# zgcr/SimpleAICV_pytorch_training_examples

Measured on AMD Instinct MI355X. Metric: training images/sec/node, higher is better.
Workload: dtype bf16; 1 GPU; resnet50 3x224x224 synthetic training step (fwd+loss+bwd+all-reduce+optimizer), per-GPU batch 256; model=resnet50, global_batch=256, per_gpu_batch=256, parallelism=dp1, step_graph=True, bn_statistics=fixed-order partial rows, deterministic=True, loop=tools.scripts.train_classification, optimizer=SGD, param_groups=2

## Files before the change

### include/saicv_hip.h

```cpp
#ifndef SAICV_HIP_H
#define SAICV_HIP_H

#include <stddef.h>
#include <stdint.h>

#ifdef __cplusplus
extern "C" {
#endif

#define SAICV_BF16 0
#define SAICV_F32 1

typedef struct saicv_conv_desc {
    int N, H, W, C;
    int K, R, S;
    int stride, pad;
    int OH, OW;
    int dtype;
} saicv_conv_desc;

int saicv_version(void);
const char* saicv_last_error_string(void);

int saicv_set_deterministic(int on);
// ... 43 lines not shown
int saicv_linear_gelu_fwd_aux(int dtype, const void* x, const void* wf, const float* bias, void* y_dact, void* y_act, int M,
                              int K, int N, void* stream);
int saicv_linear_dgrad_mul(int dtype, const void* dy, const void* wd, const void* factor, void* dx, int M, int K, int N,
                           void* stream);
int saicv_linear_wgrad(int dtype, const void* dy, const void* x, float* dw, float* dbias, int M, int K, int N,
                       void* stream);
int saicv_conv2d_dgrad_add(const saicv_conv_desc* d, const void* dy, const void* wd, const void* addend, void* dx,
                           void* stream);
typedef struct saicv_dgrad_fuse {
    const void* addend;
    const void* addend_gate;
    const void* bn_y;
    const void* bn_mask;
    const float* bn_mean;
    const float* bn_invstd;
    float* part_g;
    float* part_gx;
    int part_rows;
    int reserved;
} saicv_dgrad_fuse;
int saicv_conv2d_dgrad_stat_rows(const saicv_conv_desc* d);
int saicv_conv2d_dgrad_fused(const saicv_conv_desc* d, const void* dy, const void* wd, const saicv_dgrad_fuse* f, void* dx,
                             void* stream);
#define SAICV_PLAN_CONV_FWD 0
#define SAICV_PLAN_CONV_DGRAD 1
#define SAICV_PLAN_CONV_WGRAD 2
#define SAICV_PLAN_LINEAR_FWD 3
#define SAICV_PLAN_LINEAR_DGRAD 4
#define SAICV_PLAN_LINEAR_WGRAD 5
typedef struct saicv_plan_query {
    int op;
    saicv_conv_desc conv;
    int dtype, M, K, N;
    int out_f32, bias, stats, addend, row_scale, bn_sums, act_mode;
} saicv_plan_query;
#define SAICV_ROUTE_TILED 0
#define SAICV_ROUTE_PW_STREAM 1
#define SAICV_ROUTE_PW3_STREAM 2
#define SAICV_ROUTE_TN 3
typedef struct saicv_plan {
    int route;
    int tile;
    int bm, bn;
    int kc8;
    int plain;
    int out_f32;
// ... 275 lines not shown
```

### simpleaicv_pytorch_training_examples_amd/_lib.py

```python
import ctypes
import os
from ctypes import POINTER, Structure, c_char_p, c_double, c_float, c_int, c_long, c_size_t, c_void_p

import torch

HERE = os.path.dirname(os.path.abspath(__file__))
LIB_PATH = os.path.join(HERE, 'libsaicv_hip.so')

BF16, F32 = 0, 1


class ConvDesc(Structure):
    _fields_ = [('N', c_int), ('H', c_int), ('W', c_int), ('C', c_int), ('K', c_int), ('R', c_int),
                ('S', c_int), ('stride', c_int), ('pad', c_int), ('OH', c_int), ('OW', c_int),
                ('dtype', c_int)]


_P = c_void_p
_PD = POINTER(ConvDesc)


class AttnDesc(Structure):
    _fields_ = [('q', _P), ('k', _P), ('v', _P),
                ('q_rs', c_long), ('k_rs', c_long), ('v_rs', c_long),
# ... 53 lines not shown
    'saicv_last_error_string': (c_char_p, []),
    'saicv_set_deterministic': (c_int, [c_int]),
    'saicv_get_deterministic': (c_int, []),
    'saicv_deterministic_prepare': (c_int, [_P]),
    'saicv_pack_input': (c_int, [c_int, _P, c_long, c_long, c_long, c_long, _P, c_int, c_int, c_int, c_int, c_int, _P]),
    'saicv_pack_weight': (c_int, [c_int, _P, c_long, c_long, c_long, c_long, c_int, c_int, c_int, c_int, c_int, c_int, _P, _P, _P]),
    'saicv_unpack_wgrad': (c_int, [_P, c_int, c_int, c_int, c_int, c_int, _P, c_long, c_long, c_long, c_long, c_int, _P]),
    'saicv_pack_weight_batched': (c_int, [c_int, _P, c_int, c_int, _P]),
    'saicv_pack_input_s2d': (c_int, [c_int, _P, c_long, c_long, c_long, c_long, _P, c_int, c_int, c_int, c_int, c_int, c_int, _P]),
    'saicv_pack_weight_s2d': (c_int, [c_int, _P, c_long, c_long, c_long, c_long, c_int, c_int, c_int, c_int, c_int, _P, _P]),
    'saicv_unpack_wgrad_s2d': (c_int, [_P, c_int, c_int, c_int, c_int, c_int, _P, c_long, c_long, c_long, c_long, c_int, _P]),
    'saicv_conv2d_stat_rows': (c_int, [_PD]),
    'saicv_conv2d_fwd': (c_int, [_PD, _P, _P, _P, _P, c_int, _P, _P, _P]),
    'saicv_conv2d_dgrad': (c_int, [_PD, _P, _P, _P, _P]),
    'saicv_conv2d_wgrad': (c_int, [_PD, _P, _P, _P, _P]),
    'saicv_conv2d_wgrad_bias': (c_int, [_PD, _P, _P, _P, _P, _P]),
    'saicv_colsum': (c_int, [c_int, _P, c_int, c_int, _P, _P]),
    'saicv_linear_fwd': (c_int, [c_int, _P, _P, _P, _P, c_int, c_int, c_int, c_int, _P, _P, c_int, _P]),
    'saicv_linear_dgrad': (c_int, [c_int, _P, _P, _P, c_int, c_int, c_int, _P, _P]),
    'saicv_linear_wgrad': (c_int, [c_int, _P, _P, _P, _P, c_int, c_int, c_int, _P]),
    'saicv_conv2d_dgrad_add': (c_int, [_PD, _P, _P, _P, _P, _P]),
    'saicv_conv2d_dgrad_stat_rows': (c_int, [_PD]),
    'saicv_conv2d_dgrad_fused': (c_int, [_PD, _P, _P, _PF, _P, _P]),
    'saicv_igemm_plan': (c_int, [POINTER(PlanQuery), POINTER(Plan)]),
    'saicv_conv2d_fwd_stats': (c_int, [_PD, _P, _P, _P, _P, _P, c_int, _P]),
    'saicv_bn_act_fwd_stats': (c_int, [c_int, _P, _P, _P, _P, _P, c_int, c_double, _P, _P, _P, _P, c_double, c_double, _P, _P, _P,
                                       c_size_t, c_int, c_int, _P, _P]),
    'saicv_bn_act_fwd_join': (c_int, [c_int, _P, _P, _P, _P, _P, _P, _P, _P, _P, c_int, c_double, _P, _P, _P, _P, c_double, c_double,
                                      _P, _P, _P, c_size_t, c_int, c_int, _P, _P]),
    'saicv_bn_act_bwd_inline': (c_int, [c_int, _P, _P, _P, _P, _P, _P, _P, _P, c_int, _P, _P, _P, _P, c_size_t, c_int, c_int,
                                        c_int, _P]),
    'saicv_bn_act_bwd_from_partials': (c_int, [c_int, _P, _P, _P, _P, _P, _P, _P, _P, c_int, _P, _P, _P, _P, c_size_t, c_int,
                                               c_int, c_int, _P, _P]),
    'saicv_row_scale': (c_int, [c_int, _P, _P, _P, c_size_t, c_int, c_int, _P]),
    'saicv_bn_ws_floats': (c_size_t, [c_int]),
    'saicv_bn_finalize_fwd': (c_int, [_P, _P, c_int, c_int, c_double, _P, _P, _P, _P, c_double, c_double, _P, _P, _P, _P, _P, _P, _P]),
    'saicv_bn_eval_coeffs': (c_int, [c_int, _P, _P, _P, _P, c_double, _P, _P, _P]),
    'saicv_bn_act_fwd': (c_int, [c_int, _P, _P, _P, _P, _P, c_size_t, c_int, c_int, _P, _P]),
    'saicv_bn_bwd_ws_floats': (c_size_t, [c_size_t, c_int, c_int]),
    'saicv_bn_act_bwd': (c_int, [c_int, _P, _P, _P, _P, _P, _P, _P, _P, _P, _P, _P, c_size_t, c_int, c_int, c_int, _P, _P]),
    'saicv_maxpool_fwd': (c_int, [c_int, _P, _P, _P, c_int, c_int, c_int, c_int, c_int, c_int, c_int, c_int, c_int, _P]),
    'saicv_maxpool_bwd': (c_int, [c_int, _P, _P, _P, c_int, c_int, c_int, c_int, c_int, c_int, c_int, c_int, c_int, _P]),
    'saicv_bn_relu_maxpool_fwd': (c_int, [c_int, _P, _P, _P, _P, _P] + [c_int] * 9 + [_P]),
    'saicv_bn_relu_maxpool_bwd_ws_floats': (c_size_t, [c_int]),
    'saicv_bn_relu_maxpool_bwd': (c_int, [c_int, _P, _P, _P, _P, _P, _P, _P, _P, _P, _P, _P, c_int, _P] + [c_int] * 9 + [_P]),
    'saicv_avgpool_fwd': (c_int, [c_int, _P, _P, c_int, c_int, c_int, _P]),
# ... 162 lines not shown
```

### simpleaicv_pytorch_training_examples_amd/build.py

```python
import os
import subprocess
import sys

HERE = os.path.dirname(os.path.abspath(__file__))
CSRC = os.path.join(HERE, 'csrc')
LIB = os.path.join(HERE, 'libsaicv_hip.so')
SOURCES = ['igemm.hip', 'pwstream.hip', 'bn.hip', 'pool.hip', 'loss.hip', 'pack.hip', 'optim.hip', 'muon.hip', 'tfm.hip', 'attn_stream.hip', 'maskloss.hip', 'sam.hip', 'samtail.hip', 'semseg.hip', 'salient.hip', 'input.hip', 'dwconv.hip', 'elemwise.hip', 'detloss.hip', 'groupnorm.hip', 'comm.hip', 'det.hip', 'capi.hip']
FLAGS = ['--offload-arch=gfx950', '-O3', '-std=c++17', '-fPIC', '-munsafe-fp-atomics',
         '-Wno-unused-result', '-Wno-unused-value']
EXTRA_FLAGS = {'attn_stream.hip': ['-fno-honor-nans', '-Wno-inline-asm']}


def _hipcc():
    for cand in (os.environ.get('HIPCC'), '/opt/rocm/bin/hipcc', 'hipcc'):
        if cand and (os.path.isabs(cand) and os.path.exists(cand) or not os.path.isabs(cand)):
            return cand
    return 'hipcc'


def _stale(out, deps):
    if not os.path.exists(out):
        return True
    t = os.path.getmtime(out)
    return any(os.path.getmtime(d) > t for d in deps if os.path.exists(d))


def build(force=False, verbose=True):
    hipcc = _hipcc()
    headers = [os.path.join(CSRC, h) for h in os.listdir(CSRC) if h.endswith('.h')]
    headers.append(os.path.join(os.path.dirname(HERE), 'include', 'saicv_hip.h'))
# ... 35 lines not shown
```

### simpleaicv_pytorch_training_examples_amd/csrc/bn.hip

```cpp
#include "common.h"
#include "saicv_internal.h"

namespace {


constexpr int kMaxBlocks = 1024;

__global__ __launch_bounds__(256) void bn_reduce_partials_kernel(const float* __restrict__ a,
                                                                 const float* __restrict__ b, int P,
                                                                 int C, float* __restrict__ oa,
                                                                 float* __restrict__ ob, int rows_per) {
    const int c = blockIdx.x * 64 + (threadIdx.x & 63);
    const int ty = threadIdx.x >> 6;
    const int p0 = blockIdx.y * rows_per;
    const int p1 = min(P, p0 + rows_per);
    float sa = 0.f, sb = 0.f;
    if (c < C) {
        float a4[4] = {0.f, 0.f, 0.f, 0.f}, b4[4] = {0.f, 0.f, 0.f, 0.f};
        int p = p0 + ty;
        for (; p + 12 < p1; p += 16) {
#pragma unroll
            for (int u = 0; u < 4; ++u) {
                a4[u] += a[(size_t)(p + 4 * u) * C + c];
                b4[u] += b[(size_t)(p + 4 * u) * C + c];
// ... 553 lines not shown
    SAICV_REQUIRE(part_g && part_gx && rows >= 1 && rows <= 64, "bn_bwd_inline: partial sums missing");
    SAICV_REQUIRE(!relu || relu_mask != nullptr, "bn_bwd_inline: relu needs the sign mask");
    const BnBwdInline inl = {part_g, part_gx, rows, (float)M, gamma, mean, invstd, dgamma, dbeta, accumulate};
    if (dtype == SAICV_DTYPE_BF16) return bn_bwd_inline_t<bf16_t>(dz, (const uint8_t*)relu_mask, y, dy, dres, M, C, relu, inl, st);
    return bn_bwd_inline_t<float>(dz, (const uint8_t*)relu_mask, y, dy, dres, M, C, relu, inl, st);
}

int bn_bwd_from_partials(int dtype, const void* dz, const void* relu_mask, const void* y, const float* gamma,
                         const float* mean, const float* invstd, const float* part_g, const float* part_gx, int rows,
                         void* dy, void* dres, float* dgamma, float* dbeta, size_t M, int C, int relu, int accumulate,
                         float* ws, hipStream_t st) {
    const uint8_t* mask = (const uint8_t*)relu_mask;
    const int n = dtype == SAICV_DTYPE_BF16 ? 8 : 4;
    SAICV_REQUIRE(C % n == 0, "bn_bwd_from_partials: C=%d must be a multiple of %d", C, n);
    SAICV_REQUIRE(part_g != nullptr && part_gx != nullptr && rows > 0, "bn_bwd_from_partials: partial sums missing");
    SAICV_REQUIRE(!relu || mask != nullptr, "bn_bwd_from_partials: relu needs the sign mask");
    if (dtype == SAICV_DTYPE_BF16)
        return bn_bwd_t<bf16_t>(dz, nullptr, mask, y, gamma, mean, invstd, dy, dres, dgamma, dbeta, M, C, relu, accumulate, ws, st,
                                part_g, part_gx, rows);
    return bn_bwd_t<float>(dz, nullptr, mask, y, gamma, mean, invstd, dy, dres, dgamma, dbeta, M, C, relu, accumulate, ws, st,
                           part_g, part_gx, rows);
}

int bn_bwd(int dtype, const void* dz, const void* z, const void* relu_mask, const void* y, const float* gamma,
           const float* mean, const float* invstd, void* dy, void* dres, float* dgamma, float* dbeta,
           size_t M, int C, int relu, int accumulate, float* ws, hipStream_t st) {
    const uint8_t* mask = (const uint8_t*)relu_mask;
    const int n = dtype == SAICV_DTYPE_BF16 ? 8 : 4;
    SAICV_REQUIRE(C % n == 0, "bn_bwd: C=%d must be a multiple of %d", C, n);
    SAICV_REQUIRE(!relu || z != nullptr || mask != nullptr, "bn_bwd: relu needs the forward output z or its sign mask");
    if (dtype == SAICV_DTYPE_BF16)
        return bn_bwd_t<bf16_t>(dz, z, mask, y, gamma, mean, invstd, dy, dres, dgamma, dbeta, M, C, relu, accumulate, ws, st);
    return bn_bwd_t<float>(dz, z, mask, y, gamma, mean, invstd, dy, dres, dgamma, dbeta, M, C, relu, accumulate, ws, st);
}

}
```

### simpleaicv_pytorch_training_examples_amd/csrc/capi.hip

```cpp
#include <stdarg.h>
#include <stdio.h>
#include <string.h>

#include "common.h"
#include "saicv_internal.h"
#include "../../include/saicv_hip.h"

namespace saicv {

static thread_local char g_err[512] = "";

void set_error(const char* fmt, ...) {
    va_list ap;
    va_start(ap, fmt);
    vsnprintf(g_err, sizeof(g_err), fmt, ap);
    va_end(ap);
}

int check_launch(const char* what) {
    const hipError_t e = hipGetLastError();
    if (e != hipSuccess) {
        set_error("%s: launch failed: %s", what, hipGetErrorString(e));
        return -2;
    }
// ... 216 lines not shown
                             void* stream) {
    if (check_desc(d, "saicv_conv2d_dgrad_fused")) return -1;
    if (!f) { set_error("saicv_conv2d_dgrad_fused: null fusion descriptor"); return -1; }
    const int M = d->N * d->H * d->W;
    EpiExtra ex;
    ex.addend = f->addend;
    ex.addend_gate = static_cast<const uint8_t*>(f->addend_gate);
    ex.bs_y = f->bn_y;
    ex.bs_mask = static_cast<const uint8_t*>(f->bn_mask);
    ex.bs_mean = f->bn_mean;
    ex.bs_invstd = f->bn_invstd;
    ex.bs_g = f->part_g;
    ex.bs_gx = f->part_gx;
    ex.stat_atomic_rows = f->part_rows;
    if (f->bn_y && d->stride > 1 && f->part_rows == 0) {
        const size_t bytes = (size_t)saicv_conv2d_dgrad_stat_rows(d) * d->C * sizeof(float);
        if (f->part_g) hipMemsetAsync(f->part_g, 0, bytes, S(stream));
        if (f->part_gx) hipMemsetAsync(f->part_gx, 0, bytes, S(stream));
    }
    return igemm_nt(d->dtype, 1, dy, wd, dx, nullptr, nullptr, nullptr, d->OH, d->OW, d->K, d->H, d->W,
                    d->R, d->S, d->stride, d->pad, M, d->C, d->R * d->S * d->K, d->C, 0, S(stream),
                    (f->addend || f->bn_y) ? &ex : nullptr);
}
int saicv_igemm_plan(const saicv_plan_query* q, saicv_plan* plan) {
    if (!q || !plan) { set_error("saicv_igemm_plan: null argument"); return -1; }
    SAICV_REQUIRE(q->op >= SAICV_PLAN_CONV_FWD && q->op <= SAICV_PLAN_LINEAR_WGRAD, "saicv_igemm_plan: bad op %d", q->op);
    if (q->op <= SAICV_PLAN_CONV_WGRAD) {
        if (check_desc(&q->conv, "saicv_igemm_plan")) return -1;
    } else {
        SAICV_REQUIRE(q->dtype == SAICV_BF16 || q->dtype == SAICV_F32, "saicv_igemm_plan: bad dtype %d", q->dtype);
    }
    return igemm_plan(q, plan);
}
int saicv_row_scale(int dtype, const void* x, const float* scale, void* out, size_t rows, int row_len,
                    int rows_per_scale, void* stream) {
    return row_scale(dtype, x, scale, out, rows, row_len, rows_per_scale, S(stream));
}

int saicv_colsum(int dtype, const void* dy, int M, int N, float* dbias, void* stream) {
    return colsum(dtype, dy, M, N, dbias, S(stream));
}

size_t saicv_bn_ws_floats(int C) { return bn_ws_floats(C); }

int saicv_bn_finalize_fwd(const float* sum, const float* sq, int rows, int C, double count,
                          const float* gamma, const float* beta, float* running_mean,
// ... 291 lines not shown
```

### simpleaicv_pytorch_training_examples_amd/csrc/saicv_internal.h

```cpp
#pragma once
#include <hip/hip_runtime.h>

struct saicv_conv_desc;
struct saicv_plan_query;
struct saicv_plan;

namespace saicv {

void set_error(const char* fmt, ...);
int check_launch(const char* what);

int conv_stat_rows(const saicv_conv_desc* d);
struct EpiExtra {
    const void* addend = nullptr;
    const float* row_scale = nullptr;
    int rows_per_scale = 1;
    int act_mode = 0;
    void* out2 = nullptr;
    const uint8_t* addend_gate = nullptr;
    const void* bs_y = nullptr;
    const uint8_t* bs_mask = nullptr;
    const float* bs_mean = nullptr;
    const float* bs_invstd = nullptr;
    float* bs_g = nullptr;
    float* bs_gx = nullptr;
    int stat_atomic_rows = 0;
};
int conv_bwd_stat_rows(const saicv_conv_desc* d);
int igemm_nt(int dtype, int mode, const void* src, const void* wgt, void* out, const float* bias,
             float* stat_sum, float* stat_sq, int H, int W, int C, int OH, int OW, int R, int S,
             int stride, int pad, int M, int Nn, int Kd, int ldo, int out_f32, hipStream_t st,
             const EpiExtra* ex = nullptr);
int igemm_tn(int dtype, const void* dy, const void* src, float* dw, int H, int W, int C, int OH,
             int OW, int R, int S, int stride, int pad, int M, int Cout, int Kd, hipStream_t st,
             float* dbias = nullptr);

int igemm_plan(const saicv_plan_query* q, saicv_plan* out);

int pw_stream_blocks(int dtype, int M, int Nn, int Kd, bool fused_dgrad);
int pw_stream(int M, int Nn, int Kd, const void* src, const void* wgt, void* out, float* stat_sum, float* stat_sq,
              int stat_atomic_rows, const EpiExtra* ex, int stream_out, int blocks, hipStream_t st);
int pw3_stream_blocks(int dtype, int M, int Nn, int Kd);
int pw3_stream(int mode, int M, int H, int W, const void* src, const void* wgt, void* out, float* stat_sum, float* stat_sq,
               int stat_atomic_rows, const EpiExtra* ex, int stream_out, int blocks, hipStream_t st);

int window_partition(int dtype, const void* x, void* out, int B, int H, int W, int C, int ws, hipStream_t st);
int window_unpartition(int dtype, const void* win, const void* addend, void* out, int B, int H, int W, int C, int ws,
                       hipStream_t st);
int relpos_fwd(int dtype, const void* q, long q_rs, long q_bs, const float* tab_h, const float* tab_w, float* rel_h,
               float* rel_w, int B, int heads, int Sh, int Sw, hipStream_t st);
int relpos_bwd(int dtype, const void* q, void* dq, long q_rs, long q_bs, const float* tab_h, const float* tab_w,
               const float* d_rel_h, const float* d_rel_w, float* dtab_h, float* dtab_w, float* ws, int B, int heads, int Sh,
               int Sw, hipStream_t st);
size_t relpos_bwd_ws_floats(int Sh, int Sw);
int mask_loss_stats(int dtype, const void* logits, const float* targets, float* stats, int B, int M, size_t HW,
                    double alpha, double gamma, double thr, hipStream_t st);
int mask_loss_grad(int dtype, const void* logits, const float* targets, const float* coef, void* dlogits, int B, int M,
                   size_t HW, double alpha, double gamma, hipStream_t st);
int hyper_product_fwd(int dtype, const void* x, const void* hyper, void* out, int B, int Tm, int P, int C, hipStream_t st);
int hyper_product_bwd(int dtype, const void* x, const void* hyper, const void* dout, void* dx, float* dhyper, int B, int Tm,
                      int P, int C, hipStream_t st);
int upsample4_fwd(int dtype, const void* low, void* out, int planes, int h, int w, hipStream_t st);
int upsample4_bwd(int dtype, const void* dhi, void* dlow, int planes, int h, int w, hipStream_t st);
int mask_loss_stats_up4(int dtype, const void* low, const float* targets, float* stats, int B, int M, int h, int w,
                        double alpha, double gamma, double thr, hipStream_t st);
int mask_loss_grad_up4(int dtype, const void* low, const float* targets, const float* coef, void* dlow, int B, int M, int h,
                       int w, double alpha, double gamma, hipStream_t st);
size_t pixel_softmax_ce_ws_floats(size_t rows);
// ... 19 lines not shown
```

### simpleaicv_pytorch_training_examples_amd/ops.py

```python
import collections
import ctypes
import weakref

import torch

from . import _lib
from ._lib import ConvDesc, check, dtype_code, lib, ptr, require_gpu, stream

_weights_epoch = [0]


class KernelTimer:
    enabled = False
    only = None
    records = []
    PEAK_FLOPS, PEAK_BYTES = 2.5e15, 8.0e12

    @classmethod
    def begin(cls, tag=None):
        if not cls.enabled or (cls.only is not None and tag not in cls.only):
            return None
        e = torch.cuda.Event(enable_timing=True)
        e.record()
        return e
# ... 688 lines not shown
        fuse.bn_mean, fuse.bn_invstd = ptr(in_link.mean), ptr(in_link.invstd)
        fuse.part_g, fuse.part_gx = ptr(part[0]), ptr(part[1])
        in_link.part, in_link.rows = part, rows
    return fuse


def _pooled_bn_backward(ctx, st, dz, gamma, y, idx, mean, invstd):
    pk, ps, pp, poh, pow_, scale, shift = ctx.pool
    L = lib()
    dt, dev = y.dtype, y.device
    n, k, oh, ow = y.shape
    dy = _empty_nhwc(n, k, oh, ow, dt, dev)
    dgamma, dbeta, direct_bn = _bn_grad_buffers(gamma, ctx.beta_ref, k, dev)
    ws = torch.empty(L.saicv_bn_relu_maxpool_bwd_ws_floats(k), dtype=torch.float32, device=dev)
    t0 = KernelTimer.begin('bn_act_bwd')
    check(L.saicv_bn_relu_maxpool_bwd(dtype_code(dt), ptr(dz), ptr(idx), ptr(y), ptr(gamma), ptr(mean), ptr(invstd), ptr(scale),
                                      ptr(shift), ptr(dy), ptr(dgamma), ptr(dbeta), int(direct_bn), ptr(ws), n, oh, ow, k, poh, pow_,
                                      pk, ps, pp, st), 'bn_relu_maxpool_bwd')
    es = y.element_size()
    KernelTimer.end(t0, 'bn_act_bwd', 0, 3.0 * n * oh * ow * k * es + 2.0 * n * poh * pow_ * k * (es + 1))
    return (dy, None, None, None) if direct_bn else (dy, None, dgamma, dbeta)


class ConvBnActFn(torch.autograd.Function):

    _deferred = []

    @staticmethod
    def forward(ctx, x, weight, gamma, beta, residual, bn, stride, pad, relu, want_skip=False, pool=None, defer=False):
        if defer and (residual is not None or relu or want_skip or pool is not None):
            raise ValueError('a deferred BatchNorm-apply belongs to a plain convolution + BatchNorm shortcut')
        if pool is not None and (residual is not None or not relu or want_skip):
            raise ValueError('the fused max-pool follows a plain conv -> BatchNorm -> ReLU block')
        cs = _conv_stage(x, weight, gamma, beta, bn, stride, pad, ctx.needs_input_grad[0], pool is not None, defer)
        if pool is not None:
            return _pooled_tail(ctx, cs, weight, gamma, beta, stride, pad, pool)
        if defer:
            _remember(ctx, cs, weight, gamma, beta, stride, pad, False, False, applies_gate=bool(BN_FUSE and cs.training))
            ConvBnActFn._deferred.append((cs.scale, cs.shift))
            return cs.y
        return _apply_tail(ctx, cs, weight, gamma, beta, stride, pad, relu, residual, want_skip)

    @staticmethod
    def backward(ctx, dz, dskip=None):
        x, weight, gamma, y, mask, mean, invstd = ctx.saved_tensors
        stride, pad, relu, has_res, training, d, wd = ctx.cfg
        if not training:
            raise NotImplementedError('backward through eval-mode BatchNorm is not implemented')
        dt, st = y.dtype, stream()
        gate_in = _take_gate(dz)
        dz0 = dz
        dz = _nhwc(dz, dt)
        if ctx.pool is not None:
            dy, dres, dgamma, dbeta = _pooled_bn_backward(ctx, st, dz, gamma, y, mask, mean, invstd)
        else:
            dy, dres, dgamma, dbeta = _bn_act_backward(ctx, st, dz, dz is dz0, gate_in, relu, has_res, gamma, y, mask, mean, invstd)
        n, k, oh, ow = y.shape
        M = n * oh * ow
        c = x.shape[1]
        flops = 2.0 * M * k * weight.shape[2] * weight.shape[3] * min(c, weight.shape[1])
        dx = dwt = None
        if ctx.needs_input_grad[0]:
            t0 = KernelTimer.begin('igemm_nt')
            gate = None
            if dskip is not None:
                gate = _take_gate(dskip)
                dskip = _nhwc(dskip, dt)
            in_link = ctx.in_link
            fuse = _dgrad_fuse(d, in_link, dskip, gate, y.device) if (gate is not None or in_link is not None) else None
            dx = _conv_data_grad(d, dy, weight, wd, x.shape, dt, st, fuse, dskip)
            if in_link is not None:
                in_link.dx, in_link.dx_version = dx, dx._version
            es = dy.element_size()
            px = float(n) * x.shape[2] * x.shape[3] * c
            nbytes = float(M) * k * es + float(k) * d.R * d.S * c * es + px * es
# ... 855 lines not shown
```

Baseline: 12550 images/s.

## Fuse bottleneck conv3 backward: BN-ReLU grad, dgrad and wgrad in one streaming kernel

Adds a streaming kernel for the 1x1 expansion conv of residual bottlenecks. In a single pass over each tile it applies the BN/ReLU backward coefficients to dz, computes the data gradient and accumulates the weight gradient, and optionally produces the next BN's partial sums. This removes separate BN-backward, dgrad and wgrad launches, along with the round trip of the intermediate dy tensor through memory. The trade-offs are a narrow eligibility condition, heavy register and LDS use per workgroup, and a deterministic cross-block reduction of the weight gradient.

```diff
diff --git a/include/saicv_hip.h b/include/saicv_hip.h
--- a/include/saicv_hip.h
+++ b/include/saicv_hip.h
@@ -89,6 +89,13 @@
 int saicv_conv2d_dgrad_stat_rows(const saicv_conv_desc* d);
 int saicv_conv2d_dgrad_fused(const saicv_conv_desc* d, const void* dy, const void* wd, const saicv_dgrad_fuse* f, void* dx,
                              void* stream);
+int saicv_c3_bwd_stream_ok(int dtype, int M, int CO, int CI);
+int saicv_c3_bwd_stream_rows(int M, int CO, int CI);
+size_t saicv_c3_bwd_stream_ws_floats(int M, int CO, int CI);
+int saicv_c3_bwd_stream(int dtype, const void* dz, const void* relu_mask, const void* y, const float* gamma, const float* mean,
+                        const float* invstd, const float* part_g, const float* part_gx, int rows, float* dgamma, float* dbeta,
+                        int accumulate, float* ws, const void* x, const void* wd, const saicv_dgrad_fuse* f, void* dx, float* dw,
+                        int M, int CO, int CI, void* stream);
 #define SAICV_PLAN_CONV_FWD 0
 #define SAICV_PLAN_CONV_DGRAD 1
 #define SAICV_PLAN_CONV_WGRAD 2
diff --git a/simpleaicv_pytorch_training_examples_amd/_lib.py b/simpleaicv_pytorch_training_examples_amd/_lib.py
--- a/simpleaicv_pytorch_training_examples_amd/_lib.py
+++ b/simpleaicv_pytorch_training_examples_amd/_lib.py
@@ -99,6 +99,10 @@
     'saicv_conv2d_dgrad_add': (c_int, [_PD, _P, _P, _P, _P, _P]),
     'saicv_conv2d_dgrad_stat_rows': (c_int, [_PD]),
     'saicv_conv2d_dgrad_fused': (c_int, [_PD, _P, _P, _PF, _P, _P]),
+    'saicv_c3_bwd_stream_ok': (c_int, [c_int, c_int, c_int, c_int]),
+    'saicv_c3_bwd_stream_rows': (c_int, [c_int, c_int, c_int]),
+    'saicv_c3_bwd_stream_ws_floats': (c_size_t, [c_int, c_int, c_int]),
+    'saicv_c3_bwd_stream': (c_int, [c_int, _P, _P, _P, _P, _P, _P, _P, _P, c_int, _P, _P, c_int, _P, _P, _P, _PF, _P, _P, c_int, c_int, c_int, _P]),
     'saicv_igemm_plan': (c_int, [POINTER(PlanQuery), POINTER(Plan)]),
     'saicv_conv2d_fwd_stats': (c_int, [_PD, _P, _P, _P, _P, _P, c_int, _P]),
     'saicv_bn_act_fwd_stats': (c_int, [c_int, _P, _P, _P, _P, _P, c_int, c_double, _P, _P, _P, _P, c_double, c_double, _P, _P, _P,
diff --git a/simpleaicv_pytorch_training_examples_amd/build.py b/simpleaicv_pytorch_training_examples_amd/build.py
--- a/simpleaicv_pytorch_training_examples_amd/build.py
+++ b/simpleaicv_pytorch_training_examples_amd/build.py
@@ -5,7 +5,7 @@
 HERE = os.path.dirname(os.path.abspath(__file__))
 CSRC = os.path.join(HERE, 'csrc')
 LIB = os.path.join(HERE, 'libsaicv_hip.so')
-SOURCES = ['igemm.hip', 'pwstream.hip', 'bn.hip', 'pool.hip', 'loss.hip', 'pack.hip', 'optim.hip', 'muon.hip', 'tfm.hip', 'attn_stream.hip', 'maskloss.hip', 'sam.hip', 'samtail.hip', 'semseg.hip', 'salient.hip', 'input.hip', 'dwconv.hip', 'elemwise.hip', 'detloss.hip', 'groupnorm.hip', 'comm.hip', 'det.hip', 'capi.hip']
+SOURCES = ['igemm.hip', 'pwstream.hip', 'c3bwd.hip', 'bn.hip', 'pool.hip', 'loss.hip', 'pack.hip', 'optim.hip', 'muon.hip', 'tfm.hip', 'attn_stream.hip', 'maskloss.hip', 'sam.hip', 'samtail.hip', 'semseg.hip', 'salient.hip', 'input.hip', 'dwconv.hip', 'elemwise.hip', 'detloss.hip', 'groupnorm.hip', 'comm.hip', 'det.hip', 'capi.hip']
 FLAGS = ['--offload-arch=gfx950', '-O3', '-std=c++17', '-fPIC', '-munsafe-fp-atomics',
          '-Wno-unused-result', '-Wno-unused-value']
 EXTRA_FLAGS = {'attn_stream.hip': ['-fno-honor-nans', '-Wno-inline-asm']}
diff --git a/simpleaicv_pytorch_training_examples_amd/csrc/bn.hip b/simpleaicv_pytorch_training_examples_amd/csrc/bn.hip
--- a/simpleaicv_pytorch_training_examples_amd/csrc/bn.hip
+++ b/simpleaicv_pytorch_training_examples_amd/csrc/bn.hip
@@ -599,6 +599,17 @@
                            part_g, part_gx, rows);
 }
 
+int bn_bwd_coeffs(const float* part_g, const float* part_gx, int rows, int C, size_t M, const float* gamma, const float* mean,
+                  const float* invstd, float* dgamma, float* dbeta, int accumulate, float* ws, hipStream_t st) {
+    SAICV_REQUIRE(part_g != nullptr && part_gx != nullptr && rows > 0 && ws != nullptr, "bn_bwd_coeffs: partial sums missing");
+    const float* a = part_g; const float* b = part_gx;
+    float* coef = ws + (size_t)64 * C;
+    const int P = reduce_partials(a, b, rows, C, ws, st);
+    hipLaunchKernelGGL(P <= 32 ? bn_finalize_bwd_kernel<4> : bn_finalize_bwd_kernel<16>, dim3((C + 63) / 64), dim3(P <= 32 ? 256 : 1024), 0, st, a, b, P, C,
+                       (float)M, gamma, mean, invstd, dgamma, dbeta, coef, coef + C, coef + 2 * C, accumulate);
+    return check_launch("bn_bwd_coeffs");
+}
+
 int bn_bwd(int dtype, const void* dz, const void* z, const void* relu_mask, const void* y, const float* gamma,
            const float* mean, const float* invstd, void* dy, void* dres, float* dgamma, float* dbeta,
            size_t M, int C, int relu, int accumulate, float* ws, hipStream_t st) {
diff --git a/simpleaicv_pytorch_training_examples_amd/csrc/c3bwd.hip b/simpleaicv_pytorch_training_examples_amd/csrc/c3bwd.hip
--- /dev/null
+++ b/simpleaicv_pytorch_training_examples_amd/csrc/c3bwd.hip
@@ -0,0 +1,420 @@
+#include <stdlib.h>
+
+#include <type_traits>
+
+#include "common.h"
+#include "det.h"
+#include "saicv_internal.h"
+#include "../../include/saicv_hip.h"
+
+namespace {
+
+struct C3Params {
+    const bf16_t* dz;
+    const bf16_t* y;
+    const uint8_t* mask;
+    const float* ca;
+    const float* cb;
+    const float* cc;
+    const bf16_t* x;
+    const bf16_t* wd;
+    bf16_t* dx;
+    float* dw;
+    const bf16_t* bs_y;
+    const uint8_t* bs_mask;
+    const float* bs_mean;
+    const float* bs_invstd;
+    float* bs_g;
+    float* bs_gx;
+    int bs_atomic_rows;
+    saicv::DetSink det;
+    uint32_t dz_bytes, mask_bytes, x_bytes;
+    int M, ntiles, tiles_per_wg;
+};
+
+DEVINL void st_plain(void* q, u32x4 v) {
+    asm volatile("global_store_dwordx4 %0, %1, off\n\ts_nop 1" ::"v"(q), "v"(v) : "memory");
+}
+template <int B, int E, typename F> DEVINL void static_for(F&& f) {
+    if constexpr (B < E) {
+        f(std::integral_constant<int, B>{});
+        static_for<B + 1, E>(f);
+    }
+}
+DEVINL int c3_key(int r) { return (r & 3) | (((r >> 3) & 1) << 2); }
+template <int CPR> DEVINL int c3_g(int r) { return CPR >= 16 ? c3_key(r) : (c3_key(r) >> 1); }
+
+constexpr int kTilePx = 32;
+constexpr size_t c3_lds_bytes(int co, int ci) {
+    return (size_t)kTilePx * (ci * 2 + 16) + (size_t)kTilePx * ci * 2 + (size_t)(co / 64) * kTilePx * 128;
+}
+
+template <int CO, int CI>
+__global__ __launch_bounds__(CO) void c3_bwd_stream_kernel(const C3Params p) {
+    constexpr int DEPTH = 2;
+    constexpr int NW = CO / 64;
+    constexpr int TP = kTilePx;
+    constexpr int XT = CI / 16;
+    constexpr int CPX = CI / 8;
+    constexpr int KSA = CO / 32;
+    constexpr int NT2 = 2 * XT / NW;
+    constexpr int OP = CI * 2 + 16;
+    constexpr int OUT_BYTES = TP * OP;
+    constexpr int XS_BYTES = TP * CI * 2;
+    constexpr uint32_t OOB = 0xfffffff0u;
+    static_assert(CO % 64 == 0 && CI % 16 == 0 && TP * CPX == CO && NT2 == 2, "one x / dx chunk per thread and tile");
+    typedef __attribute__((address_space(3))) bf16x4 lds_bf16x4;
+    extern __shared__ __attribute__((aligned(16))) char smem[];
+    char* const outt = smem;
+    char* const xs = smem + OUT_BYTES;
+    char* const strips = smem + OUT_BYTES + XS_BYTES;
+
+    const int tid = threadIdx.x;
+    const int lane = tid & 63;
+    const int wave = __builtin_amdgcn_readfirstlane(tid >> 6);
+    const int l15 = lane & 15, lg = lane >> 4;
+    const int nc0 = wave * 64;
+    char* const strip = strips + wave * (TP * 128);
+    const int opx = tid / CPX, och = tid % CPX;
+    const int mpt = wave & 1, mnt0 = (wave >> 1) * NT2;
+
+    float ka[2][8], kb[2][8], kc[2][8];
+#pragma unroll
+    for (int ks = 0; ks < 2; ++ks)
+#pragma unroll
+        for (int j = 0; j < 8; ++j) {
+            const int c = nc0 + ks * 32 + lg * 8 + j;
+            ka[ks][j] = p.ca[c]; kb[ks][j] = p.cb[c]; kc[ks][j] = p.cc[c];
+        }
+    u32x4 wf[NT2][KSA];
+#pragma unroll
+    for (int n2 = 0; n2 < NT2; ++n2)
+#pragma unroll
+        for (int ks = 0; ks < KSA; ++ks) wf[n2][ks] = ld_chunk(p.wd + (size_t)((mnt0 + n2) * 16 + l15) * CO + ks * 32 + lg * 8);
+
+    const __amdgpu_buffer_rsrc_t dz_rs = __builtin_amdgcn_make_buffer_rsrc(const_cast<bf16_t*>(p.dz), 0, p.dz_bytes, 0x00020000);
+    const __amdgpu_buffer_rsrc_t y_rs = __builtin_amdgcn_make_buffer_rsrc(const_cast<bf16_t*>(p.y), 0, p.dz_bytes, 0x00020000);
+    const __amdgpu_buffer_rsrc_t mk_rs = __builtin_amdgcn_make_buffer_rsrc(const_cast<uint8_t*>(p.mask), 0, p.mask_bytes, 0x00020000);
+    const __amdgpu_buffer_rsrc_t x_rs = __builtin_amdgcn_make_buffer_rsrc(const_cast<bf16_t*>(p.x), 0, p.x_bytes, 0x00020000);
+
+    struct Slot { u32x4 g[2][2], y[2][2]; uint32_t m[2][2]; u32x4 x; };
+    Slot slot[DEPTH];
+    const int first = (int)blockIdx.x * p.tiles_per_wg;
+    const int count = max(0, min(p.tiles_per_wg, p.ntiles - first));
+    auto tile_of = [&](int i) { return i < count ? first + i : -1; };
+    const uint32_t frag_off = ((uint32_t)l15 * CO + nc0 + lg * 8) * 2u;
+    const uint32_t xo_off = ((uint32_t)opx * CI + och * 8) * 2u;
+    auto load_tile = [&](Slot& s, int tile) __attribute__((always_inline)) {
+        const bool ok = tile >= 0;
+        const uint32_t fb = (uint32_t)tile * (TP * CO * 2) + frag_off;
+#pragma unroll
+        for (int pt = 0; pt < 2; ++pt)
+#pragma unroll
+            for (int ks = 0; ks < 2; ++ks) {
+                const uint32_t o = fb + pt * (16 * CO * 2) + ks * 64;
+                s.g[pt][ks] = __builtin_amdgcn_raw_buffer_load_b128(dz_rs, (int)(ok ? o : OOB), 0, 0);
+                s.y[pt][ks] = __builtin_amdgcn_raw_buffer_load_b128(y_rs, (int)(ok ? o : OOB), 0, 0);
+                s.m[pt][ks] = __builtin_amdgcn_raw_buffer_load_b8(mk_rs, (int)(ok ? (o >> 4) : OOB), 0, 0);
+            }
+        const uint32_t xo = (uint32_t)tile * (TP * CI * 2) + xo_off;
+        s.x = __builtin_amdgcn_raw_buffer_load_b128(x_rs, (int)(ok ? xo : OOB), 0, 0);
+    };
+#pragma unroll
+    for (int dd = 0; dd < DEPTH; ++dd) load_tile(slot[dd], tile_of(dd));
+
+    f32x4 accw[4][XT];
+#pragma unroll
+    for (int a = 0; a < 4; ++a)
+#pragma unroll
+        for (int b = 0; b < XT; ++b) accw[a][b] = f32x4{0.f, 0.f, 0.f, 0.f};
+
+    const int row0 = lg * 8 + (l15 >> 2);
+    int fa_off[4], fb_off[XT];
+#pragma unroll
+    for (int a = 0; a < 4; ++a) fa_off[a] = row0 * 128 + ((a ^ c3_g<8>(row0)) << 5) + (l15 & 3) * 8;
+#pragma unroll
+    for (int b = 0; b < XT; ++b) fb_off[b] = row0 * (CI * 2) + ((b ^ c3_g<CPX>(row0)) << 5) + (l15 & 3) * 8;
+    const int xs_off = opx * (CI * 2) + ((och ^ (c3_g<CPX>(opx) << 1)) << 4);
+    const int mrow = mpt * 16 + l15;
+    int mb_off[2];
+#pragma unroll
+    for (int k1 = 0; k1 < 2; ++k1) mb_off[k1] = mrow * 128 + (((k1 * 4 + lg) ^ (c3_g<8>(mrow) << 1)) << 4);
+
+    auto step = [&](auto D, int i) __attribute__((always_inline)) {
+        constexpr int d = decltype(D)::value;
+        Slot& s = slot[d];
+        const int tile = tile_of(i);
+#pragma unroll
+        for (int ks = 0; ks < 2; ++ks)
+#pragma unroll
+            for (int pt = 0; pt < 2; ++pt) {
+                float g[8], yy[8], o[8];
+                Chunk<bf16_t>::unpack(s.g[pt][ks], g);
+                Chunk<bf16_t>::unpack(s.y[pt][ks], yy);
+                const uint32_t bits = s.m[pt][ks];
+#pragma unroll
+                for (int j = 0; j < 8; ++j) {
+                    const float gj = ((bits >> j) & 1u) ? g[j] : 0.f;
+                    o[j] = fmaf(ka[ks][j], gj, fmaf(kb[ks][j], yy[j], kc[ks][j]));
+                }
+                const int row = pt * 16 + l15, ch = ks * 4 + lg;
+                *reinterpret_cast<u32x4*>(strip + row * 128 + ((ch ^ (c3_g<8>(row) << 1)) << 4)) = Chunk<bf16_t>::pack(o);
+            }
+        *reinterpret_cast<u32x4*>(xs + xs_off) = s.x;
+        load_tile(s, tile_of(i + DEPTH));
+        __syncthreads();
+        f32x4 acc[NT2];
+#pragma unroll
+        for (int n2 = 0; n2 < NT2; ++n2) acc[n2] = f32x4{0.f, 0.f, 0.f, 0.f};
+#pragma unroll
+        for (int ks = 0; ks < KSA; ++ks) {
+            const u32x4 bfr = ld_chunk(strips + (ks >> 1) * (TP * 128) + mb_off[ks & 1]);
+#pragma unroll
+            for (int n2 = 0; n2 < NT2; ++n2) Mma<bf16_t>::run(acc[n2], wf[n2][ks], bfr);
+        }
+#pragma unroll
+        for (int n2 = 0; n2 < NT2; ++n2) {
+            bf16x4 pk;
+#pragma unroll
+            for (int r = 0; r < 4; ++r) pk[r] = (bf16_t)acc[n2][r];
+            *reinterpret_cast<bf16x4*>(outt + mrow * OP + ((mnt0 + n2) * 16 + lg * 4) * 2) = pk;
+        }
+        {
+            u32x4 af[4], bf[XT];
+#pragma unroll
+            for (int a = 0; a < 4; ++a) {
+                const bf16x4 l4 = __builtin_amdgcn_ds_read_tr16_b64_v4bf16((lds_bf16x4*)(strip + fa_off[a]));
+                const bf16x4 h4 = __builtin_amdgcn_ds_read_tr16_b64_v4bf16((lds_bf16x4*)(strip + fa_off[a] + 4 * 128));
+                const u32x2 l2 = __builtin_bit_cast(u32x2, l4), h2 = __builtin_bit_cast(u32x2, h4);
+                af[a] = u32x4{l2[0], l2[1], h2[0], h2[1]};
+            }
+#pragma unroll
+            for (int b = 0; b < XT; ++b) {
+                const bf16x4 l4 = __builtin_amdgcn_ds_read_tr16_b64_v4bf16((lds_bf16x4*)(xs + fb_off[b]));
+                const bf16x4 h4 = __builtin_amdgcn_ds_read_tr16_b64_v4bf16((lds_bf16x4*)(xs + fb_off[b] + 4 * CI * 2));
+                const u32x2 l2 = __builtin_bit_cast(u32x2, l4), h2 = __builtin_bit_cast(u32x2, h4);
+                bf[b] = u32x4{l2[0], l2[1], h2[0], h2[1]};
+            }
+#pragma unroll
+            for (int a = 0; a < 4; ++a)
+#pragma unroll
+                for (int b = 0; b < XT; ++b) Mma<bf16_t>::run(accw[a][b], af[a], bf[b]);
+        }
+        __syncthreads();
+        {
+            const u32x4 v = ld_chunk(outt + opx * OP + och * 16);
+            const int row = tile * TP + opx;
+            if (row < p.M) st_plain(p.dx + (size_t)row * CI + och * 8, v);
+        }
+        __syncthreads();
+    };
+    int i0 = 0;
+    for (; i0 + DEPTH <= count; i0 += DEPTH) static_for<0, DEPTH>([&](auto D) { step(D, i0 + decltype(D)::value); });
+    static_for<0, DEPTH - 1>([&](auto D) {
+        if (i0 + decltype(D)::value < count) step(D, i0 + decltype(D)::value);
+    });
+
+#pragma unroll
+    for (int a = 0; a < 4; ++a)
+#pragma unroll
+        for (int b = 0; b < XT; ++b)
+#pragma unroll
+            for (int r = 0; r < 4; ++r) {
+                const size_t idx = (size_t)(nc0 + a * 16 + lg * 4 + r) * CI + b * 16 + l15;
+                saicv::det_add(p.det, p.dw + idx, idx, (int)blockIdx.x, accw[a][b][r]);
+            }
+}
+
+constexpr int bs_nwaves(int nd) { return nd / 64 > 4 ? nd / 64 : 4; }
+template <int ND>
+__global__ __launch_bounds__(64 * bs_nwaves(ND)) void c3_bs_sums_kernel(const C3Params p, int mtiles, int units) {
+    constexpr int NSPLIT = ND / 64, NWAVES = bs_nwaves(ND), GPB = NWAVES / NSPLIT;
+    constexpr int CPR = 8, RPP = 8;
+    __shared__ float red[NWAVES * 2 * 64];
+    const int lane = threadIdx.x & 63;
+    const int wave = __builtin_amdgcn_readfirstlane(threadIdx.x >> 6);
+    const int slice = wave % NSPLIT, nc0 = slice * 64;
+    const int unit = blockIdx.x * GPB + wave / NSPLIT;
+    const int U = units;
+    const int crow = lane / CPR, cchunk = lane % CPR;
+    const bool maskp = p.bs_mask != nullptr;
+    const int count = unit < mtiles ? (mtiles - unit + U - 1) / U : 0;
+    struct Ops { u32x4 v[2], y[2]; unsigned m[2]; };
+    auto load = [&](Ops& o, int i) __attribute__((always_inline)) {
+        const int tile = unit + i * U;
+#pragma unroll
+        for (int ps = 0; ps < 2; ++ps) {
+            const int row = tile * 16 + ps * RPP + crow;
+            const bool rok = i < count && row < p.M;
+            const size_t ooff = (size_t)row * ND + nc0 + cchunk * 8;
+            o.v[ps] = u32x4{0u, 0u, 0u, 0u};
+            o.y[ps] = u32x4{0u, 0u, 0u, 0u};
+            o.m[ps] = 0xffu;
+            if (rok) {
+                o.v[ps] = ld_chunk(p.dx + ooff);
+                o.y[ps] = ld_chunk(p.bs_y + ooff);
+                if (maskp) o.m[ps] = p.bs_mask[ooff >> 3];
+            }
+        }
+    };
+    float ssum[8], ssq[8];
+#pragma unroll
+    for (int e = 0; e < 8; ++e) { ssum[e] = 0.f; ssq[e] = 0.f; }
+    auto add = [&](const Ops& o) __attribute__((always_inline)) {
+#pragma unroll
+        for (int ps = 0; ps < 2; ++ps) {
+            float f[8], yy[8];
+            Chunk<bf16_t>::unpack(o.v[ps], f);
+            Chunk<bf16_t>::unpack(o.y[ps], yy);
+#pragma unroll
+            for (int e = 0; e < 8; ++e) {
+                const float ge = ((o.m[ps] >> e) & 1u) ? f[e] : 0.f;
+                ssum[e] += ge;
+                ssq[e] = fmaf(ge, yy[e], ssq[e]);
+            }
+        }
+    };
+    Ops oa, ob;
+    load(oa, 0);
+    for (int i = 0; i < count; i += 2) {
+        load(ob, i + 1);
+        add(oa);
+        load(oa, i + 2);
+        if (i + 1 < count) add(ob);
+    }
+#pragma unroll
+    for (int e = 0; e < 8; ++e) {
+        const int c = nc0 + cchunk * 8 + e;
+        ssq[e] = p.bs_invstd[c] * fmaf(-p.bs_mean[c], ssum[e], ssq[e]);
+    }
+#pragma unroll
+    for (int e = 0; e < 8; ++e) {
+        ssum[e] += __shfl_xor(ssum[e], 8, 64);  ssq[e] += __shfl_xor(ssq[e], 8, 64);
+        ssum[e] += __shfl_xor(ssum[e], 16, 64); ssq[e] += __shfl_xor(ssq[e], 16, 64);
+        ssum[e] += __shfl_xor(ssum[e], 32, 64); ssq[e] += __shfl_xor(ssq[e], 32, 64);
+    }
+    if (lane < CPR) {
+#pragma unroll
+        for (int e = 0; e < 8; ++e) {
+            red[(wave * 2 + 0) * 64 + lane * 8 + e] = ssum[e];
+            red[(wave * 2 + 1) * 64 + lane * 8 + e] = ssq[e];
+        }
+    }
+    __syncthreads();
+    const size_t row = p.bs_atomic_rows ? (size_t)(blockIdx.x % p.bs_atomic_rows) : (size_t)blockIdx.x;
+    for (int c = threadIdx.x; c < 2 * ND; c += 64 * NWAVES) {
+        const int which = c / ND, col = c - which * ND;
+        const int sl = col / 64, cc = col - sl * 64;
+        float a = 0.f;
+#pragma unroll
+        for (int g = 0; g < GPB; ++g) a += red[((g * NSPLIT + sl) * 2 + which) * 64 + cc];
+        float* dst = (which ? p.bs_gx : p.bs_g) + row * ND + col;
+        if (p.bs_atomic_rows) unsafeAtomicAdd(dst, a); else *dst = a;
+    }
+}
+
+int c3_sum_rows(int M, int ci) {
+    const int nsplit = ci / 64, nwaves = nsplit > 4 ? nsplit : 4, gpb = nwaves / nsplit;
+    const int mtiles = (M + 15) / 16, want = (mtiles + gpb - 1) / gpb, cap = 256 * 2 * 4 / nwaves;
+    return want < cap ? want : cap;
+}
+
+struct C3Shape { int co, ci; bool routed; };
+constexpr C3Shape kC3Shapes[] = {{256, 64, true}, {512, 128, false}};
+
+template <int CO, int CI>
+int launch_c3(const C3Params& p, int blocks, hipStream_t st) {
+    auto k = c3_bwd_stream_kernel<CO, CI>;
+    constexpr size_t smem = c3_lds_bytes(CO, CI);
+    static bool once = (hipFuncSetAttribute(reinterpret_cast<const void*>(k), hipFuncAttributeMaxDynamicSharedMemorySize, (int)smem), true);
+    (void)once;
+    hipLaunchKernelGGL(k, dim3(blocks), dim3(CO), smem, st, p);
+    return saicv::check_launch("c3_bwd_stream");
+}
+
+}
+
+namespace saicv {
+
+int c3_bwd_stream_rows(int M, int CO, int CI) {
+    if (M < 1 || ((size_t)M + kTilePx) * CO * 2 >= 0xfffffff0ull) return 0;
+    for (const C3Shape& s : kC3Shapes)
+        if (s.co == CO && s.ci == CI) return c3_sum_rows(M, CI);
+    return 0;
+}
+
+static int c3_plan(int M, int CO, int CI, int* splits, int* tiles_per_wg) {
+    saicv_plan_query q = {};
+    q.op = SAICV_PLAN_CONV_WGRAD;
+    q.conv.N = 1; q.conv.H = M; q.conv.W = 1; q.conv.C = CI; q.conv.K = CO; q.conv.R = 1; q.conv.S = 1; q.conv.stride = 1; q.conv.pad = 0;
+    q.conv.OH = M; q.conv.OW = 1; q.conv.dtype = SAICV_BF16;
+    saicv_plan pl;
+    if (igemm_plan(&q, &pl) != 0) return -1;
+    SAICV_REQUIRE(pl.splits >= 1 && (pl.rt_per * pl.rows_per_step) % kTilePx == 0, "c3_bwd_stream: weight-gradient plan with %d x %d rows per split",
+                  pl.rt_per, pl.rows_per_step);
+    *splits = pl.splits;
+    *tiles_per_wg = pl.rt_per * pl.rows_per_step / kTilePx;
+    return 0;
+}
+
+size_t c3_bwd_stream_ws_floats(int M, int CO, int CI) {
+    size_t n = (size_t)67 * CO;
+    int splits = 0, tpw = 0;
+    if (!g_deterministic && c3_bwd_stream_rows(M, CO, CI) > 0 && c3_plan(M, CO, CI, &splits, &tpw) == 0 && splits > 1)
+        n += (size_t)splits * CO * CI;
+    return n;
+}
+
+int c3_bwd_stream_blocks(int dtype, int M, int CO, int CI) {
+    const char* es = getenv("SAICV_C3_BWD_STREAM");
+    const char* er = getenv("SAICV_C3_BWD_MIN_ROWS");
+    const int on = es ? atoi(es) : 1;
+    const int min_rows = er ? atoi(er) : 65536;
+    if (!on || dtype != SAICV_DTYPE_BF16 || M < min_rows) return 0;
+    for (const C3Shape& s : kC3Shapes)
+        if (s.co == CO && s.ci == CI && s.routed) return c3_bwd_stream_rows(M, CO, CI);
+    return 0;
+}
+
+int c3_bwd_stream(int M, int CO, int CI, const void* dz, const void* y, const void* mask, const float* coef, const void* x,
+                  const void* wd, void* dx, float* dw, const EpiExtra* ex, int bs_rows, float* part_ws, hipStream_t st) {
+    SAICV_REQUIRE(c3_bwd_stream_rows(M, CO, CI) > 0, "c3_bwd_stream: no form for M = %d, Cout = %d, Cin = %d (bf16, (256, 64) or (512, 128), "
+                  "operands below 4 GiB)", M, CO, CI);
+    SAICV_REQUIRE(dz && y && mask && coef && x && wd && dx && dw, "c3_bwd_stream: operand missing");
+    C3Params p = {};
+    p.dz = (const bf16_t*)dz; p.y = (const bf16_t*)y; p.mask = (const uint8_t*)mask;
+    p.ca = coef; p.cb = coef + CO; p.cc = coef + 2 * CO;
+    p.x = (const bf16_t*)x; p.wd = (const bf16_t*)wd; p.dx = (bf16_t*)dx; p.dw = dw;
+    if (ex && ex->bs_y) {
+        SAICV_REQUIRE(ex->bs_mean && ex->bs_invstd && ex->bs_g && ex->bs_gx, "c3_bwd_stream: BatchNorm-backward sums need mean / invstd / outputs");
+        p.bs_y = (const bf16_t*)ex->bs_y; p.bs_mask = ex->bs_mask; p.bs_mean = ex->bs_mean; p.bs_invstd = ex->bs_invstd;
+        p.bs_g = ex->bs_g; p.bs_gx = ex->bs_gx;
+        p.bs_atomic_rows = bs_rows;
+    }
+    p.dz_bytes = (uint32_t)((size_t)M * CO * 2);
+    p.mask_bytes = (uint32_t)((size_t)M * CO / 8);
+    p.x_bytes = (uint32_t)((size_t)M * CI * 2);
+    p.M = M;
+    p.ntiles = (M + kTilePx - 1) / kTilePx;
+    int blocks = 0;
+    if (c3_plan(M, CO, CI, &blocks, &p.tiles_per_wg) != 0) return -1;
+    DetParts parts;
+    if (parts.begin(st, blocks, (size_t)CO * CI, "c3_bwd_stream", false) != 0) return -1;
+    if (!parts.on() && blocks > 1) {
+        SAICV_REQUIRE(part_ws != nullptr, "c3_bwd_stream: workspace for the weight-gradient parts missing");
+        parts.s.part = part_ws;
+    }
+    p.det = parts.sink();
+    int rc = CO == 256 ? launch_c3<256, 64>(p, blocks, st) : launch_c3<512, 128>(p, blocks, st);
+    if (rc != 0) return rc;
+    if (parts.fold(dw, 0, (size_t)CO * CI, true) != 0) return -1;
+    if (p.bs_y) {
+        const int rows = c3_sum_rows(M, CI), mtiles = (M + 15) / 16;
+        if (CI == 64) hipLaunchKernelGGL(c3_bs_sums_kernel<64>, dim3(rows), dim3(64 * bs_nwaves(64)), 0, st, p, mtiles, rows * (bs_nwaves(64) / 1));
+        else hipLaunchKernelGGL(c3_bs_sums_kernel<128>, dim3(rows), dim3(64 * bs_nwaves(128)), 0, st, p, mtiles, rows * (bs_nwaves(128) / 2));
+        return check_launch("c3_bs_sums");
+    }
+    return 0;
+}
+
+}
diff --git a/simpleaicv_pytorch_training_examples_amd/csrc/capi.hip b/simpleaicv_pytorch_training_examples_amd/csrc/capi.hip
--- a/simpleaicv_pytorch_training_examples_amd/csrc/capi.hip
+++ b/simpleaicv_pytorch_training_examples_amd/csrc/capi.hip
@@ -262,6 +262,30 @@
                     d->R, d->S, d->stride, d->pad, M, d->C, d->R * d->S * d->K, d->C, 0, S(stream),
                     (f->addend || f->bn_y) ? &ex : nullptr);
 }
+int saicv_c3_bwd_stream_ok(int dtype, int M, int CO, int CI) { return c3_bwd_stream_blocks(dtype, M, CO, CI); }
+int saicv_c3_bwd_stream_rows(int M, int CO, int CI) { return c3_bwd_stream_rows(M, CO, CI); }
+size_t saicv_c3_bwd_stream_ws_floats(int M, int CO, int CI) { return c3_bwd_stream_ws_floats(M, CO, CI); }
+int saicv_c3_bwd_stream(int dtype, const void* dz, const void* relu_mask, const void* y, const float* gamma, const float* mean,
+                        const float* invstd, const float* part_g, const float* part_gx, int rows, float* dgamma, float* dbeta,
+                        int accumulate, float* ws, const void* x, const void* wd, const saicv_dgrad_fuse* f, void* dx, float* dw,
+                        int M, int CO, int CI, void* stream) {
+    SAICV_REQUIRE(dtype == SAICV_BF16, "saicv_c3_bwd_stream: bf16 only (dtype %d)", dtype);
+    SAICV_REQUIRE(c3_bwd_stream_rows(M, CO, CI) > 0, "saicv_c3_bwd_stream: no form for M = %d, Cout = %d, Cin = %d", M, CO, CI);
+    SAICV_REQUIRE(mean && invstd && ws, "saicv_c3_bwd_stream: statistics / workspace missing");
+    SAICV_REQUIRE(!f || (!f->addend && !f->addend_gate), "saicv_c3_bwd_stream: no addend form");
+    if (bn_bwd_coeffs(part_g, part_gx, rows, CO, (size_t)M, gamma, mean, invstd, dgamma, dbeta, accumulate, ws, S(stream)) != 0) return -1;
+    EpiExtra ex;
+    if (f && f->bn_y) {
+        ex.bs_y = f->bn_y;
+        ex.bs_mask = static_cast<const uint8_t*>(f->bn_mask);
+        ex.bs_mean = f->bn_mean;
+        ex.bs_invstd = f->bn_invstd;
+        ex.bs_g = f->part_g;
+        ex.bs_gx = f->part_gx;
+    }
+    return c3_bwd_stream(M, CO, CI, dz, y, relu_mask, ws + (size_t)64 * CO, x, wd, dx, dw, (f && f->bn_y) ? &ex : nullptr,
+                         f ? f->part_rows : 0, ws + (size_t)67 * CO, S(stream));
+}
 int saicv_igemm_plan(const saicv_plan_query* q, saicv_plan* plan) {
     if (!q || !plan) { set_error("saicv_igemm_plan: null argument"); return -1; }
     SAICV_REQUIRE(q->op >= SAICV_PLAN_CONV_FWD && q->op <= SAICV_PLAN_LINEAR_WGRAD, "saicv_igemm_plan: bad op %d", q->op);
diff --git a/simpleaicv_pytorch_training_examples_amd/csrc/saicv_internal.h b/simpleaicv_pytorch_training_examples_amd/csrc/saicv_internal.h
--- a/simpleaicv_pytorch_training_examples_amd/csrc/saicv_internal.h
+++ b/simpleaicv_pytorch_training_examples_amd/csrc/saicv_internal.h
@@ -44,6 +44,14 @@
 int pw3_stream(int mode, int M, int H, int W, const void* src, const void* wgt, void* out, float* stat_sum, float* stat_sq,
                int stat_atomic_rows, const EpiExtra* ex, int stream_out, int blocks, hipStream_t st);
 
+int c3_bwd_stream_blocks(int dtype, int M, int CO, int CI);
+int c3_bwd_stream_rows(int M, int CO, int CI);
+int c3_bwd_stream(int M, int CO, int CI, const void* dz, const void* y, const void* mask, const float* coef, const void* x,
+                  const void* wd, void* dx, float* dw, const EpiExtra* ex, int bs_rows, float* part_ws, hipStream_t st);
+size_t c3_bwd_stream_ws_floats(int M, int CO, int CI);
+int bn_bwd_coeffs(const float* part_g, const float* part_gx, int rows, int C, size_t M, const float* gamma, const float* mean,
+                  const float* invstd, float* dgamma, float* dbeta, int accumulate, float* ws, hipStream_t st);
+
 int window_partition(int dtype, const void* x, void* out, int B, int H, int W, int C, int ws, hipStream_t st);
 int window_unpartition(int dtype, const void* win, const void* addend, void* out, int B, int H, int W, int C, int ws,
                        hipStream_t st);
diff --git a/simpleaicv_pytorch_training_examples_amd/ops.py b/simpleaicv_pytorch_training_examples_amd/ops.py
--- a/simpleaicv_pytorch_training_examples_amd/ops.py
+++ b/simpleaicv_pytorch_training_examples_amd/ops.py
@@ -734,6 +734,71 @@
     return (dy, None, None, None) if direct_bn else (dy, None, dgamma, dbeta)
 
 
+def _c3_fused_backward(ctx, st, dz, dz_is_given, gate_in, dskip, x, weight, gamma, y, mask, mean, invstd):
+    stride, pad, relu, has_res, training, d, wd = ctx.cfg
+    dt = y.dtype
+    if not (BN_FUSE and dt == torch.bfloat16 and relu and has_res and mask is not None and gate_in is None and dskip is None
+            and dz_is_given and ctx.s2d is None and (d.R, d.S, d.stride, d.pad) == (1, 1, 1, 0)
+            and ctx.needs_input_grad[0] and ctx.needs_input_grad[1] and (ctx.gated_res or not ctx.needs_input_grad[4])):
+        return None
+    link = ctx.link
+    if not (link is not None and link.part is not None and link.dx is not None and dz.data_ptr() == link.dx.data_ptr()
+            and dz.shape == link.dx.shape and dz._version == link.dx_version):
+        return None
+    n, k, oh, ow = y.shape
+    c = x.shape[1]
+    M = n * oh * ow
+    if c != weight.shape[1] or tuple(x.shape) != (n, c, oh, ow) or x.dtype != dt:
+        return None
+    L, dev = lib(), y.device
+    rows = L.saicv_c3_bwd_stream_ok(dtype_code(dt), M, k, c)
+    if rows <= 0:
+        return None
+    dres = None
+    if ctx.needs_input_grad[4]:
+        dres = dz
+        dres._saicv_gate = mask
+        dres._saicv_gate_version = dres._version
+        _GateLedger.hand_out()
+    dgamma, dbeta, direct_bn = _bn_grad_buffers(gamma, ctx.beta_ref, k, dev)
+    ws = torch.empty(L.saicv_c3_bwd_stream_ws_floats(M, k, c), dtype=torch.float32, device=dev)
+    if wd is None:
+        _, wd = packed_weight(weight, dt, c, True, d.K)
+    in_link = ctx.in_link
+    fuse = None
+    if in_link is not None:
+        fuse = _lib.DgradFuse()
+        in_link.inline = BN_INLINE and c <= 2048
+        if in_link.inline:
+            prow = _stat_rows(rows)
+            part = _ZeroPool.take(2 * prow * c, dev).view(2, prow, c)
+            fuse.part_rows = prow
+        else:
+            prow = rows
+            part = torch.empty((2, rows, c), dtype=torch.float32, device=dev)
+        fuse.bn_y, fuse.bn_mask = ptr(in_link.y), ptr(in_link.mask)
+        fuse.bn_mean, fuse.bn_invstd = ptr(in_link.mean), ptr(in_link.invstd)
+        fuse.part_g, fuse.part_gx = ptr(part[0]), ptr(part[1])
+        in_link.part, in_link.rows = part, prow
+    dx = _empty_nhwc(n, c, oh, ow, dt, dev)
+    gw = _arena_grad(weight)
+    direct = (gw is not None and d.K == weight.shape[0] and weight.is_contiguous(memory_format=torch.channels_last))
+    dw = gw if direct else torch.zeros((k, 1, 1, c), dtype=torch.float32, device=dev)
+    t0 = KernelTimer.begin('c3_bwd_stream')
+    check(L.saicv_c3_bwd_stream(dtype_code(dt), ptr(dz), ptr(mask), ptr(y), ptr(gamma), ptr(mean), ptr(invstd), ptr(link.part[0]),
+                                ptr(link.part[1]), link.rows, ptr(dgamma), ptr(dbeta), int(direct_bn), ptr(ws), ptr(x), ptr(wd),
+                                ctypes.byref(fuse) if fuse is not None else None, ptr(dx), ptr(dw), M, k, c, st), 'c3_bwd_stream')
+    KernelTimer.end(t0, 'c3_bwd_stream', 2 * 2.0 * M * k * c, 2.75 * M * k * y.element_size())
+    link.part = link.dx = None
+    if in_link is not None:
+        in_link.dx, in_link.dx_version = dx, dx._version
+    dwt = None if direct else _weight_grad(dw, weight, c)
+    if direct_bn:
+        dgamma = dbeta = None
+    return (dx, dwt, dgamma if ctx.needs_input_grad[2] else None, dbeta if ctx.needs_input_grad[3] else None, dres,
+            None, None, None, None, None, None, None)
+
+
 class ConvBnActFn(torch.autograd.Function):
 
     _deferred = []
@@ -763,6 +828,10 @@
         gate_in = _take_gate(dz)
         dz0 = dz
         dz = _nhwc(dz, dt)
+        if ctx.pool is None:
+            fused = _c3_fused_backward(ctx, st, dz, dz is dz0, gate_in, dskip, x, weight, gamma, y, mask, mean, invstd)
+            if fused is not None:
+                return fused
         if ctx.pool is not None:
             dy, dres, dgamma, dbeta = _pooled_bn_backward(ctx, st, dz, gamma, y, mask, mean, invstd)
         else:
```

Result: faster. 12890 images/s (median of 6 runs) (+2.7%).
